# FlowEternal/multitask-hydranet

Hardware: AMD Instinct MI355X
Metric: images/sec (fwd+bwd) HydraNet @ default res, 1/2/4/8 MI355X; CPU-ref same run (higher is better)
Workload: dtype bf16; 1 GPU; full HydraNet (backbone + BiFPN + seg/det/lane heads + multitask loss), big cfg, fwd+loss+bwd; batch_per_gpu=16, global_batch=16, resolution=3x512x1024, parallelism=dp1, hipgraph=True

## Files before the change

### include/hydranet_hip.h

```cpp
#ifndef HYDRANET_HIP_H
#define HYDRANET_HIP_H

#ifdef __cplusplus
extern "C" {
#endif

typedef struct ihipStream_t* hipStream_t;


int hn_gconv_pack_diag(const float* w, void* wk, void* wd, int C, hipStream_t stream);
int hn_pack_weight(const float* w, void* wp, void* wt, int Cout, int Cin, int taps, hipStream_t stream);
int hn_pack_weight_ex(const float* w, void* wp, void* wt, int Cout, int Cin_total, int ci0, int Cin, int taps, int phase, const float* bias,
                      float* b_eff, hipStream_t stream);
int hn_phase_fold(const float* dw_eff, const float* dw1, const float* db_eff, float* dw, float* db, int K, int C0, int C1, hipStream_t stream);
int hn_pack_weights_batched(const long* jobs, int njobs, long total_blocks, const int* block_job, hipStream_t stream);
int hn_pack_small_batched(const long* jobs, const int* block_job, long total_blocks, hipStream_t stream);

int hn_conv_gemm_nt(const void* x0, const void* x1, int mode, int n_img, int H, int W, int C0, int C1, int ld0, int ld1, int up, long M,
                    const void* w, int Nout, int KP, int taps, const float* bias, int act, void* out, int out_f32, int ldc, long rpi,
                    long img_stride, float* psum, float* psq, hipStream_t stream);
int hn_nt_stat_rows(long M, int Nout);
int hn_nt_stat_tile(long M, int Nout);
int hn_conv_gemm_nt_stream(const void* x, int ld0, long M, int C0, const void* w, int Nout, int KP, const float* bias, int act, void* out,
                           int ldc, float* psum, float* psq, int wg_limit, hipStream_t stream);
int hn_nt_stream_ok(long M, int C0, int Nout, int KP);
int hn_direct_stat_rows(int n_img, int H, int W);
int hn_conv_gemm_nt_imgw(const void* x0, int ld0, long M, int C0, const void* w, long w_img_stride, long rows_per_image, int Nout, int KP,
                         const float* bias, int act, void* out, int ldc, const void* addend, int ld_add, hipStream_t stream);
int hn_scale_weight_gate(const void* wp, const float* gate, void* out, int N, int Cout, int C, int KP, hipStream_t stream);
int hn_conv_gemm_nt_lvl(const void* x0, int ld0, long M, int C0, const void* w, int Nout, int KP, const float* bias, int act, void* out,
                        int ldc, const float* coef, int nlev, const long* rows, hipStream_t stream);
int hn_conv_gemm_nt_lvlout(const void* x0, int ld0, long M, int C0, const void* w, int Nout, int KP, const float* bias, int act, float* out,
                           int ldc, long img_stride, int n_img, int nlev, const int* H, const int* W, int row_align, hipStream_t stream);

int hn_conv_gemm_nt_ex(const void* x0, const void* x1, int mode, int n_img, int H, int W, int C0, int C1, int ld0, int ld1, int up, long M,
                       const void* w, int Nout, int KP, int taps, const float* bias, int act, void* out, int out_f32, int ldc, long rpi,
                       long img_stride, float* psum, float* psq, const float* xscale, const float* xshift, const float* xgate, long xhw,
                       int xact, const void* addend, int ld_add, int add_mode, hipStream_t stream);
int hn_conv_gemm_nt_stat(const void* x0, const void* x1, int mode, int n_img, int H, int W, int C0, int C1, int ld0, int ld1, int up, long M,
                         const void* w, int Nout, int KP, int taps, const float* bias, int act, void* out, int out_f32, int ldc, long rpi,
                         long img_stride, float* psum, float* psq, const void* addend, int ld_add, int add_mode, int emode, const void* ez,
                         int ld_ez, const float* ecoef, hipStream_t stream);
int hn_conv_gemm_nt_stat3(const void* x0, int ld0, long M, int C0, const void* w, int Nout, int KP, void* out, int ldc, float* psum, float* psq,
                          const void* addend, int ld_add, const void* ez, int ld_ez, const void* ey, int ld_ey, const float* ecoef,
                          hipStream_t stream);
int hn_wgrad_plan(int mode, int n_img, int H, int W, long M, int Nout, int KP, int taps, int* splits, long* rows_per_split, long* ws_bytes);
int hn_conv_gemm_tn(const void* x0, const void* x1, int mode, int n_img, int H, int W, int C0, int C1, int ld0, int ld1, int up, long M,
                    const void* dz, int ldz, int Nout, int KP, int taps, float* workspace, float* dw, hipStream_t stream);


int hn_stem_fwd(const float* x, const float* w, void* z, void* patches, int N, int H, int W, hipStream_t stream);

int hn_gconv_pack(const float* w, void* wk, void* wd, int C, int flip, hipStream_t stream);
int hn_gconv_fwd(const void* in, int ldi, const void* wk, void* out, int ldo, int N, int Hi, int Wi, int C, int stride, hipStream_t stream);
int hn_gconv_dgrad_s2(const void* dz, int ldz, const void* wd, void* dx, int ldx, int N, int Hi, int Wi, int C, hipStream_t stream);
long hn_wgrad_chunks(long pixels, long items);
int hn_gconv_wgrad(const void* x, int ldx, const void* dz, int ldz, float* part, int N, int Hi, int Wi, int C, int stride,
                   hipStream_t stream);

int hn_dw_pack(const float* w, void* wk, void* wkf, int C, hipStream_t stream);
int hn_dwconv_fwd(const void* in, int ldi, const void* wk, void* out, int ldo, int N, int H, int W, int C, hipStream_t stream);
int hn_dwconv_fwd_levels(const void* in, int ldi, const void* wk, void* out, int ldo, int N, int C, int nlev, const int* H, const int* W,
                         int row_align, int accumulate, hipStream_t stream);
long hn_dwconv_wgrad_blocks(long strips, int C);
int hn_dwconv_wgrad(const void* x, int ldx, const void* dz, int ldz, float* part, int N, int H, int W, int C, hipStream_t stream);
int hn_dwconv_wgrad_levels(const void* x, int ldx, const void* dz, int ldz, float* part, int N, int C, int nlev, const int* H, const int* W,
                           int row_align, hipStream_t stream);
long hn_dwconv_bwd_blocks(long strips, int C);
long hn_dwconv_bwd_blocks_levels(int N, int C, int nlev, const int* H, const int* W);
int hn_dwconv_bwd_levels(const void* dz, int ldz, const void* x, int ldx, const void* wf, void* dx, int lddx, float* part, int N, int C,
                         int nlev, const int* H, const int* W, int row_align, int accumulate, hipStream_t stream);

int hn_maxpool_fwd(const void* in, int ldi, void* out, int ldo, int N, int H, int W, int C, int mode, hipStream_t stream);
int hn_maxpool_bwd(const void* in, int ldi, const void* dout, int ldd, void* dx, int ldx, const float* wscale, int N, int H, int W, int C,
                   int mode, hipStream_t stream);
int hn_maxpool_bwd2(const void* in, int ldi, const void* dout, int ldd, void* dx, int ldx, const float* wscale, void* arg_ws, int N, int H,
                    int W, int C, int mode, int accumulate, hipStream_t stream);

int hn_up2_fwd(const void* in, int ldi, void* out, int ldo, int N, int H, int W, int C, hipStream_t stream);
int hn_sum2x2(const void* g, int ldg, void* out, int ldo, const float* wscale, int N, int H, int W, int C, int accumulate, hipStream_t stream);

int hn_fuse_dweights(const float* pw, int blocks, const float* praw, int nw, float eps, float* dp, hipStream_t stream);
int hn_fuse_fwd(const void* const* in, const int* ld, const int* mode, const float* w, void* out, int ldo, int N, int H, int W, int C,
                hipStream_t stream);
int hn_fuse_fwd_raw(const void* const* in, const int* ld, const int* mode, const float* praw, int nw, float eps, float* wn, void* out, int ldo,
                    int N, int H, int W, int C, hipStream_t stream);
int hn_fuse_bwd_blocks(int N, int H, int W, int C);
int hn_fuse_bwd(const void* const* in, const int* ld, const int* mode, const float* w, const void* dout, int ldd, void* g, int ldg,
                void* const* din, const int* ldin, const int* acc, float* pw, int N, int H, int W, int C, hipStream_t stream);
int hn_fuse_bwd_arg(const void* const* in, const int* ld, const int* mode, const float* w, const void* dout, int ldd, void* g, int ldg,
                    void* const* din, const int* ldin, const int* acc, float* pw, void* const* arg_out, int N, int H, int W, int C,
                    hipStream_t stream);
int hn_maxpool_bwd_from_arg(const void* arg, const void* dout, int ldd, void* dx, int ldx, const float* wscale, int N, int H, int W, int C,
                            int mode, int accumulate, hipStream_t stream);

long hn_fold_ring_rows(int H, int W);
int hn_conv3x3_dgrad_fold(const void* dz, int ldz, int Cz, int n_img, int H, int W, const void* wt, int Nout, int KP, int phase_k, int clamp,
                          void* out, int ldo, const void* yprev, int ldy, void* ring, hipStream_t stream);
int hn_conv3x3_dgrad_fold_s2d(const void* dz, int ldz, int Cz, int n_img, int H, int W, const void* wt, int Nout, int KP, int phase_k, int clamp,
                              void* out, int ldo, void* out_s2d, int ld_s2d, const void* yprev, int ldy, void* ring, hipStream_t stream);
int hn_seg_fold(const void* dvp, int ldv, int c0, void* out, int ldo, const void* yprev, int ldy, int N, int H, int W, int C, int up,
                hipStream_t stream);

int hn_space_to_depth(const float* dy, void* out, int ldo, int N, int h, int w, int k, hipStream_t stream);

int hn_space_to_depth_blocks(int N, int h, int w, int k);
int hn_space_to_depth_bf16(const void* in, int ldi, void* out, int N, int h, int w, int k, float* psum, hipStream_t stream);

int hn_conv3x3_phase(const void* x0, int mode, int n_img, int H, int W, int C0, int ld0, const void* w, int Nout, int KP, const float* bias,
                     int act, void* out, int ldc, int k, const void* addend, int ld_add, hipStream_t stream);
int hn_conv3x3_out_argmax(const void* x0, int n_img, int H, int W, int C0, int ld0, const void* w, int k, int KP, const float* bias, long* mask,
                          hipStream_t stream);
int hn_wgrad_plan_phase(int n_img, int H, int W, int Nout, int KP, int phase_span, int* splits, long* rows_per_split, long* ws_bytes);
int hn_conv_gemm_tn_phase(const void* x0, int n_img, int H, int W, int C0, int ld0, const void* dz, int ldz, int Nout, int KP, int phase_span,
                          float* workspace, float* dw, float* dbias_eff, hipStream_t stream);
int hn_conv_gemm_tn_deferred(const void* x0, const void* x1, int mode, int n_img, int H, int W, int C0, int C1, int ld0, int ld1, int up, long M,
                             const void* dz, int ldz, int Nout, int KP, int taps, float* workspace, float* dw, long* job, hipStream_t stream);
int hn_wgrad_reduce_jobs(const long* jobs, int njobs, hipStream_t stream);
long hn_gconv_wgrad_group_ws_bytes(const long* jobs, int njobs);
int hn_gconv_wgrad_group(const long* jobs, int njobs, float* workspace, hipStream_t stream);

int hn_grad_tail(const long* jobs, int njobs, hipStream_t stream);

long hn_wgrad_group_ws_bytes(const long* jobs, int njobs);
int hn_wgrad_group(const long* jobs, int njobs, float* workspace, hipStream_t stream);

int hn_conv_gemm_tn_bias(const void* x0, const void* x1, int mode, int n_img, int H, int W, int C0, int C1, int ld0, int ld1, int up, long M,
                         const void* dz, int ldz, int Nout, int KP, int taps, float* workspace, float* dw, float* dbias, hipStream_t stream);

int hn_head_grad(const float* dy, const float* y, long rpi, long img_stride, int lds, int Nout, void* dz, int ldz, long M, int sigmoid,
                 hipStream_t stream);

int hn_pack_levels(const void* const* src, const int* ld, void* dst, int ldd, int N, int C, int nlev, const int* H, const int* W, int row_align,
                   hipStream_t stream);
int hn_head_grad_levels(const float* dy, const float* y, long img_stride, int lds, int Nout, void* dz, int ldz, int N, int nlev, const int* H,
                        const int* W, int row_align, int sigmoid, hipStream_t stream);


long hn_colred_rows(long M, long align);
int hn_col_stats(const void* x, int ldx, long M, int C, long R, float* psum, float* psq, hipStream_t stream);
int hn_col_dot(const void* a, int lda, const void* b, int ldb, long M, int C, long R, float* pdot, float* psum, hipStream_t stream);
int hn_rows_reduce(const float* in, float* out, int G, int S, int C, float alpha, hipStream_t stream);
int hn_rows_reduce2(const float* in1, const float* in2, float* out1, float* out2, int rows, int G, int C, hipStream_t stream);

int hn_bn_finalize(const float* psum, const float* psq, int prows, int C, long count, const float* gamma, const float* beta, float eps,
                   float momentum, float* running_mean, float* running_var, float* scale, float* shift, float* mean, float* rstd,
                   hipStream_t stream);
int hn_bn_eval_coeff(const float* gamma, const float* beta, const float* rm, const float* rv, float eps, int C, float* scale, float* shift,
                     hipStream_t stream);
int hn_bn_act(const void* z, int ldz, const float* scale, const float* shift, const void* res, int ldr, const float* rscale,
              const float* rshift, int act, void* out, int ldo, long M, int C, hipStream_t stream);
int hn_bn_bwd_reduce(const void* dout, int ldd, const void* z, int ldz, const void* y, int ldy, const float* scale, const float* shift,
                     const float* mean, const float* rstd, int act, long M, int C, long R, float* pg, float* pgx, hipStream_t stream);
int hn_bn_bwd_finalize(const float* pg, const float* pgx, int prows, int C, long count, float* dgamma, float* dbeta, float* mg, float* mgx,
// ... 301 lines not shown
```

### multitask_hydranet_amd/csrc/hn_stencil.hip

```cpp
#include "hn_common.h"

__global__ __launch_bounds__(256) void stem_fwd_kernel(const float* x, const float* w, bf16* z, bf16* patches, int N, int H, int W) {
    const int bidx = xcd_remap(blockIdx.x, gridDim.x);
    __shared__ float sw[27][32];
    for (int i = threadIdx.x; i < 27 * 32; i += 256) {
        const int co = i & 31, t = i >> 5;
        sw[t][co] = w[co * 27 + t];
    }
    __syncthreads();
    const int Ho = H >> 1, Wo = W >> 1, Wp = (Wo + 1) >> 1;
    const long total = (long)N * Ho * Wp;
    const long idx = (long)bidx * 256 + threadIdx.x;
    if (idx >= total) return;
    const int ox = (int)(idx % Wp) * 2;
    const long t1 = idx / Wp;
    const int oy = (int)(t1 % Ho);
    const long n = t1 / Ho;
    const bool two = ox + 1 < Wo;
    float acc[2][32];
#pragma unroll
    for (int c = 0; c < 32; ++c) { acc[0][c] = 0.f; acc[1][c] = 0.f; }
    __shared__ __attribute__((aligned(16))) bf16 sp[2][256][36];
    bf16* prow = patches ? sp[0][threadIdx.x] : nullptr;
    constexpr int PH = 256 * 36;
// ... 780 lines not shown
            const int px = (int)(((unsigned)e * magic) >> 16), pc = e - px * C8;
            const int py = px / 18, pxx = px - py * 18;
            const int iy = oy0 - 1 + py, ix = ox0 - 1 + pxx;
            const bf16* src = (px < ZPX && iy >= 0 && iy < H && ix >= 0 && ix < W) ? dz + (row0 + (long)iy * W + ix) * ldz + pc * 8 : st_zero_piece;
            st_glds16(src, sZ + ch * 1024);
        }
        for (int ch = wave; ch < XCH; ch += 4) {
            const int e = ch * 64 + lane;
            const int px = (int)(((unsigned)e * magic) >> 16), pc = e - px * C8;
            const int iy = oy0 + (px >> 4), ix = ox0 + (px & 15);
            const bf16* src = (px < XPX && iy < H && ix < W) ? x + (row0 + (long)iy * W + ix) * ldx + pc * 8 : st_zero_piece;
            st_glds16(src, sX + ch * 1024);
        }
        asm volatile("s_waitcnt vmcnt(0)" ::: "memory");
        __syncthreads();
        if (active)
#pragma unroll 1
        for (int col = colh; col < 16; col += 8) {
            bf16x4 win[3][3];
            auto load_row = [&](int py, bf16x4 (&w3)[3]) {
#pragma unroll
                for (int j = 0; j < 3; ++j) w3[j] = *reinterpret_cast<const bf16x4*>(sZ + ((py * 18 + col + j) * C4 + cq) * 8);
            };
            load_row(0, win[0]);
            load_row(1, win[1]);
#pragma unroll 1
            for (int r3 = 0; r3 < TH; r3 += 3)
#pragma unroll
            for (int rq = 0; rq < 3; ++rq) {
                const int r = r3 + rq;
                if (r >= TH) break;
                load_row(r + 2, win[(rq + 2) % 3]);
                const bf16x4 xb = *reinterpret_cast<const bf16x4*>(sX + ((r * 16 + col) * C4 + cq) * 8);
                float xv[4], da[4];
#pragma unroll
                for (int k = 0; k < 4; ++k) { xv[k] = bf2f(xb[k]); da[k] = 0.f; }
#pragma unroll
                for (int rr = 0; rr < 3; ++rr)
#pragma unroll
                    for (int j = 0; j < 3; ++j) {
                        const bf16x4 zq = win[(rq + rr) % 3][j];
#pragma unroll
                        for (int k = 0; k < 4; ++k) {
                            const float zf = bf2f(zq[k]);
                            if (HAS_DX) da[k] = fmaf(zf, wr[rr * 3 + j][k], da[k]);
                            acc[8 - (rr * 3 + j)][k] = fmaf(xv[k], zf, acc[8 - (rr * 3 + j)][k]);
                        }
                    }
                if (HAS_DX && oy0 + r < H && ox0 + col < W) {
                    bf16* dst = dx + (row0 + (long)(oy0 + r) * W + ox0 + col) * lddx + cq * 4;
                    bf16x4 v;
                    if (accumulate) {
                        const bf16x4 prev = ld4(dst);
#pragma unroll
                        for (int k = 0; k < 4; ++k) v[k] = f2bf(da[k] + bf2f(prev[k]));
                    } else {
#pragma unroll
                        for (int k = 0; k < 4; ++k) v[k] = f2bf(da[k]);
                    }
                    *reinterpret_cast<bf16x4*>(dst) = v;
                }
            }
        }
    }
    __syncthreads();
    float* red = reinterpret_cast<float*>(smem);
    if (active) {
#pragma unroll
        for (int tq = 0; tq < 9; ++tq)
#pragma unroll
            for (int k = 0; k < 4; ++k) red[(colh * C4 + cq) * 37 + tq * 4 + k] = acc[tq][k];
    }
    __syncthreads();
    float* dst = part + (long)bidx * C * 9;
    for (int o = tid; o < C4 * 36; o += 256) {
        const int g = o / 36, v = o - g * 36;
        float sum = 0.f;
#pragma unroll
        for (int c2 = 0; c2 < 8; ++c2) sum += red[(c2 * C4 + g) * 37 + v];
        dst[(long)(g * 4 + (v & 3)) * 9 + (v >> 2)] = sum;
    }
}

__global__ void dw_pack_kernel(const float* w, bf16* wk, bf16* wkf, int C) {
    const int idx = blockIdx.x * blockDim.x + threadIdx.x;
    if (idx >= 9 * C) return;
    const int c = idx % C, tap = idx / C;
    const bf16 v = f2bf(w[c * 9 + tap]);
    wk[idx] = v;
    if (wkf) wkf[(8 - tap) * C + c] = v;
}

__device__ __forceinline__ void pool_window(const bf16* in, int ldi, long n, int H, int W, int oy, int ox, int c, int mode, float* best,
                                            int* arg) {
#pragma unroll
    for (int k = 0; k < 8; ++k) { best[k] = -INFINITY; arg[k] = -1; }
    const int off = mode ? -1 : 0;
#pragma unroll
    for (int ky = 0; ky < 3; ++ky)
#pragma unroll
        for (int kx = 0; kx < 3; ++kx) {
            const int iy = 2 * oy + ky + off, ix = 2 * ox + kx + off;
            const bool inside = iy >= 0 && iy < H && ix >= 0 && ix < W;
            if (!inside && mode) continue;
            bf16x8 v = inside ? ld8(in + ((n * H + iy) * (long)W + ix) * ldi + c) : zero8();
#pragma unroll
            for (int k = 0; k < 8; ++k) {
                const float f = bf2f(v[k]);
                if (f > best[k]) { best[k] = f; arg[k] = inside ? ky * 3 + kx : 9; }
            }
        }
}

__global__ __launch_bounds__(256) void maxpool_fwd_kernel(const bf16* in, int ldi, bf16* out, int ldo, int N, int H, int W, int C,
                                                          int mode) {
    const int bidx = xcd_remap(blockIdx.x, gridDim.x);
    const int C8 = C >> 3, Ho = H >> 1, Wo = W >> 1;
    const long total = (long)N * Ho * Wo * C8;
    for (long idx = (long)bidx * 256 + threadIdx.x; idx < total; idx += (long)gridDim.x * 256) {
        const int cg = (int)(idx % C8);
        long t = idx / C8;
        const int ox = (int)(t % Wo);
        t /= Wo;
        const int oy = (int)(t % Ho);
        const long n = t / Ho;
        float best[8];
        int arg[8];
        pool_window(in, ldi, n, H, W, oy, ox, cg * 8, mode, best, arg);
        bf16x8 v;
#pragma unroll
        for (int k = 0; k < 8; ++k) v[k] = f2bf(best[k]);
        st8(out + ((n * Ho + oy) * (long)Wo + ox) * ldo + cg * 8, v);
    }
}

__global__ __launch_bounds__(256) void maxpool_bwd_kernel(const bf16* in, int ldi, const bf16* dout, int ldd, bf16* dx, int ldx,
                                                          const float* wscale, int N, int H, int W, int C, int mode) {
    const int bidx = xcd_remap(blockIdx.x, gridDim.x);
    const int C8 = C >> 3, Ho = H >> 1, Wo = W >> 1;
    const long total = (long)N * H * W * C8;
    const float ws = wscale ? *wscale : 1.0f;
    const int off = mode ? -1 : 0;
    for (long idx = (long)bidx * 256 + threadIdx.x; idx < total; idx += (long)gridDim.x * 256) {
        const int cg = (int)(idx % C8);
        long t = idx / C8;
        const int ix = (int)(t % W);
        t /= W;
        const int iy = (int)(t % H);
        const long n = t / H;
        float acc[8];
#pragma unroll
        for (int k = 0; k < 8; ++k) acc[k] = 0.f;
        for (int oy = (iy - off - 2 + 1) >> 1; 2 * oy + off <= iy; ++oy) {
            if (oy < 0 || oy >= Ho) continue;
            for (int ox = (ix - off - 2 + 1) >> 1; 2 * ox + off <= ix; ++ox) {
                if (ox < 0 || ox >= Wo) continue;
                float best[8];
                int arg[8];
                pool_window(in, ldi, n, H, W, oy, ox, cg * 8, mode, best, arg);
                const int mine = (iy - 2 * oy - off) * 3 + (ix - 2 * ox - off);
                const bf16x8 g = ld8(dout + ((n * Ho + oy) * (long)Wo + ox) * ldd + cg * 8);
#pragma unroll
                for (int k = 0; k < 8; ++k)
                    if (arg[k] == mine) acc[k] += bf2f(g[k]);
            }
        }
// ... 667 lines not shown
    const int lanes = 256 / (C >> 2);
    const long tb = g_hn_knob[7] > 0 ? g_hn_knob[7] : 768;
    long spl = (strips + (tb - 1) * lanes) / (tb * lanes);
    if (spl < 2) spl = 2;
    return (strips + spl * lanes - 1) / (spl * lanes);
}
extern "C" long hn_dwconv_bwd_blocks(long strips, int C) { return dwconv_bwd_strip_blocks(strips, C); }
static size_t dwconv_bwd_tiled_lds(int C8) {
    return (size_t)((((DWT_TH + 2) * 18 * C8 + 63) >> 6) + ((DWT_TH * 16 * C8 + 63) >> 6)) * 1024;
}
static bool dwconv_bwd_tiled_plan(int N, int C, const Levels& L, DwTiles& T, int& tpw, long& blocks) {
    T.tile_off[0] = 0;
    for (int l = 0; l < L.n; ++l) {
        T.ty[l] = (L.H[l] + DWT_TH - 1) / DWT_TH;
        T.tx[l] = (L.W[l] + 15) >> 4;
        T.tile_off[l + 1] = T.tile_off[l] + (long)N * T.ty[l] * T.tx[l];
    }
    const long total = T.tile_off[L.n];
    const int C8 = C >> 3;
    const size_t lds = dwconv_bwd_tiled_lds(C8);
#ifdef HN_NO_DW_TILED
    return false;
#endif
    if (g_hn_knob[7] < 0 || C8 > 16 || lds > 80 * 1024 || total < 512) return false;
    tpw = (int)((total + 511) / 512);
    blocks = (total + tpw - 1) / tpw;
    return true;
}
extern "C" long hn_dwconv_bwd_blocks_levels(int N, int C, int nlev, const int* H, const int* W) {
    Levels L;
    if (fill_levels(L, N, nlev, H, W) != HN_OK || (C & 7) || C < 8) return -1;
    DwTiles T;
    int tpw = 0;
    long blocks = 0;
    if (dwconv_bwd_tiled_plan(N, C, L, T, tpw, blocks)) return blocks;
    long strips = 0;
    for (int l = 0; l < nlev; ++l) strips += (long)N * H[l] * ((W[l] + 3) >> 2);
    return dwconv_bwd_strip_blocks(strips, C);
}
extern "C" int hn_dwconv_bwd_levels(const void* dz, int ldz, const void* x, int ldx, const void* wf, void* dx, int lddx, float* part, int N, int C,
                                    int nlev, const int* H, const int* W, int row_align, int accumulate, hipStream_t st) {
    Levels L;
    const int rc = fill_levels(L, N, nlev, H, W, row_align);
    if (rc != HN_OK) return rc;
    HN_CHECK_ARG(dz && x && part && (!dx || wf) && (C & 7) == 0 && C >= 8 && C <= 1024 && ((ldz | ldx) & 7) == 0 && (!dx || (lddx & 7) == 0));
    long pad_items = 0;
    if (dx && !accumulate)
        for (int l = 0; l < L.n; ++l) pad_items += (L.row_off[l + 1] - L.row_off[l] - (long)N * L.H[l] * L.W[l]) * (C >> 3);
    DwTiles T;
    int tpw = 0;
    long tblocks = 0;
    if (dwconv_bwd_tiled_plan(N, C, L, T, tpw, tblocks)) {
        const int C8 = C >> 3;
        const size_t lds = dwconv_bwd_tiled_lds(C8);
        if (lds > 64 * 1024) {
            static std::atomic<unsigned long long> optin_t{0};
            if (!lds_optin(optin_t, {(const void*)dwconv_bwd_tiled_kernel<true>, (const void*)dwconv_bwd_tiled_kernel<false>})) return HN_ERR_LAUNCH;
        }
        L.work_off[0] = 0;
        if (dx)
            hipLaunchKernelGGL(dwconv_bwd_tiled_kernel<true>, dim3((unsigned)(tblocks + cdiv(pad_items, 256))), dim3(256), lds, st, (const bf16*)dz,
                               ldz, (const bf16*)x, ldx, (const bf16*)wf, (bf16*)dx, lddx, part, N, C, tpw, (int)tblocks, L, T, accumulate);
        else
            hipLaunchKernelGGL(dwconv_bwd_tiled_kernel<false>, dim3((unsigned)tblocks), dim3(256), lds, st, (const bf16*)dz, ldz, (const bf16*)x, ldx,
                               (const bf16*)wf, (bf16*)dx, lddx, part, N, C, tpw, (int)tblocks, L, T, accumulate);
        HN_LAUNCH_CHECK();
    }
    L.work_off[0] = 0;
    for (int l = 0; l < L.n; ++l) L.work_off[l + 1] = L.work_off[l] + (long)N * L.H[l] * ((L.W[l] + 3) >> 2);
    const long strips = L.work_off[L.n];
    const int lanes = 256 / (C >> 2);
    const long blocks = dwconv_bwd_strip_blocks(strips, C);
    const int spl = (int)((strips + blocks * lanes - 1) / (blocks * lanes));
    const size_t lds = (256 * 37 + 9 * (size_t)C) * sizeof(float);
    if (lds > 64 * 1024) {
        static std::atomic<unsigned long long> optin{0};
        if (!lds_optin(optin, {(const void*)dwconv_bwd_kernel})) return HN_ERR_LAUNCH;
    }
    hipLaunchKernelGGL(dwconv_bwd_kernel, dim3((unsigned)(blocks + cdiv(pad_items, 256))), dim3(256), lds, st, (const bf16*)dz, ldz, (const bf16*)x,
                       ldx, (const bf16*)wf, (bf16*)dx, lddx, part, N, C, spl, blocks, L, accumulate);
    HN_LAUNCH_CHECK();
}

extern "C" int hn_maxpool_fwd(const void* in, int ldi, void* out, int ldo, int N, int H, int W, int C, int mode, hipStream_t st) {
    HN_CHECK_ARG(in && out && (C & 7) == 0 && ((ldi | ldo) & 7) == 0 && !(H & 1) && !(W & 1) && (mode == 0 || mode == 1));
    hipLaunchKernelGGL(maxpool_fwd_kernel, dim3(ew_grid((long)N * (H >> 1) * (W >> 1) * (C >> 3))), dim3(256), 0, st, (const bf16*)in, ldi,
                       (bf16*)out, ldo, N, H, W, C, mode);
    HN_LAUNCH_CHECK();
}
extern "C" int hn_maxpool_bwd(const void* in, int ldi, const void* dout, int ldd, void* dx, int ldx, const float* wscale, int N, int H,
                              int W, int C, int mode, hipStream_t st) {
    HN_CHECK_ARG(in && dout && dx && (C & 7) == 0 && ((ldi | ldd | ldx) & 7) == 0 && !(H & 1) && !(W & 1));
    hipLaunchKernelGGL(maxpool_bwd_kernel, dim3(ew_grid((long)N * H * W * (C >> 3))), dim3(256), 0, st, (const bf16*)in, ldi,
                       (const bf16*)dout, ldd, (bf16*)dx, ldx, wscale, N, H, W, C, mode);
    HN_LAUNCH_CHECK();
}
extern "C" int hn_maxpool_bwd2(const void* in, int ldi, const void* dout, int ldd, void* dx, int ldx, const float* wscale, void* arg_ws,
                               int N, int H, int W, int C, int mode, int accumulate, hipStream_t st) {
    HN_CHECK_ARG(in && dout && dx && arg_ws && (C & 7) == 0 && ((ldi | ldd | ldx) & 7) == 0 && !(H & 1) && !(W & 1));
    hipLaunchKernelGGL(maxpool_arg_kernel, dim3(ew_grid((long)N * (H >> 1) * (W >> 1) * (C >> 3))), dim3(256), 0, st, (const bf16*)in, ldi,
                       (unsigned char*)arg_ws, N, H, W, C, mode);
    hipLaunchKernelGGL(maxpool_bwd_arg_kernel, dim3(ew_grid((long)N * H * W * (C >> 3))), dim3(256), 0, st, (const unsigned char*)arg_ws,
                       (const bf16*)dout, ldd, (bf16*)dx, ldx, wscale, N, H, W, C, mode, accumulate);
    HN_LAUNCH_CHECK();
}
extern "C" int hn_maxpool_bwd_from_arg(const void* arg, const void* dout, int ldd, void* dx, int ldx, const float* wscale, int N, int H, int W,
                                       int C, int mode, int accumulate, hipStream_t st) {
    HN_CHECK_ARG(arg && dout && dx && (C & 7) == 0 && ((ldd | ldx) & 7) == 0 && !(H & 1) && !(W & 1));
    hipLaunchKernelGGL(maxpool_bwd_arg_kernel, dim3(ew_grid((long)N * H * W * (C >> 3))), dim3(256), 0, st, (const unsigned char*)arg,
                       (const bf16*)dout, ldd, (bf16*)dx, ldx, wscale, N, H, W, C, mode, accumulate);
    HN_LAUNCH_CHECK();
}
extern "C" int hn_up2_fwd(const void* in, int ldi, void* out, int ldo, int N, int H, int W, int C, hipStream_t st) {
    HN_CHECK_ARG(in && out && (C & 7) == 0 && ((ldi | ldo) & 7) == 0);
    hipLaunchKernelGGL(up2_fwd_kernel, dim3(ew_grid((long)N * 4 * H * W * (C >> 3))), dim3(256), 0, st, (const bf16*)in, ldi, (bf16*)out, ldo,
                       N, H, W, C);
    HN_LAUNCH_CHECK();
}
extern "C" int hn_sum2x2(const void* g, int ldg, void* out, int ldo, const float* wscale, int N, int H, int W, int C, int accumulate,
                         hipStream_t st) {
    HN_CHECK_ARG(g && out && (C & 7) == 0 && ((ldg | ldo) & 7) == 0);
    hipLaunchKernelGGL(sum2x2_kernel, dim3(ew_grid((long)N * H * W * (C >> 3))), dim3(256), 0, st, (const bf16*)g, ldg, (bf16*)out, ldo, wscale,
                       N, H, W, C, accumulate);
    HN_LAUNCH_CHECK();
}

static int fill_fuse(Fuse& f, const void* const* in, const int* ld, const int* mode, const float* w, void* out, int ldo, int N, int H,
                     int W, int C) {
    HN_CHECK_ARG(in && ld && mode && (C & 7) == 0 && (ldo & 7) == 0);
    for (int i = 0; i < 3; ++i) {
        f.in[i] = (const bf16*)in[i]; f.ld[i] = ld[i]; f.mode[i] = mode[i];
        HN_CHECK_ARG(mode[i] >= 0 && mode[i] <= 3 && (mode[i] == 0 || (in[i] && (ld[i] & 7) == 0)));
        HN_CHECK_ARG(mode[i] != 2 || (!(H & 1) && !(W & 1)));
    }
    f.w = w; f.out = (bf16*)out; f.ldo = ldo; f.N = N; f.H = H; f.W = W; f.C = C;
    f.praw = nullptr; f.nw = 0; f.eps = 0.f; f.wn = nullptr;
    return HN_OK;
}
extern "C" int hn_fuse_fwd(const void* const* in, const int* ld, const int* mode, const float* w, void* out, int ldo, int N, int H, int W,
                           int C, hipStream_t st) {
    Fuse f;
    HN_CHECK_ARG(out);
    const int rc = fill_fuse(f, in, ld, mode, w, out, ldo, N, H, W, C);
    if (rc) return rc;
    hipLaunchKernelGGL(fuse_fwd_kernel, dim3(ew_grid((long)N * H * W * (C >> 3))), dim3(256), 0, st, f);
    HN_LAUNCH_CHECK();
}
extern "C" int hn_fuse_fwd_raw(const void* const* in, const int* ld, const int* mode, const float* praw, int nw, float eps, float* wn,
                               void* out, int ldo, int N, int H, int W, int C, hipStream_t st) {
    Fuse f;
    HN_CHECK_ARG(out && praw && wn && nw >= 1 && nw <= 3);
    const int rc = fill_fuse(f, in, ld, mode, nullptr, out, ldo, N, H, W, C);
    if (rc) return rc;
    f.praw = praw; f.nw = nw; f.eps = eps; f.wn = wn;
    hipLaunchKernelGGL(fuse_fwd_kernel, dim3(ew_grid((long)N * H * W * (C >> 3))), dim3(256), 0, st, f);
    HN_LAUNCH_CHECK();
}
extern "C" int hn_fuse_bwd_blocks(int N, int H, int W, int C) {
    long b = ((long)N * H * W * (C >> 3) + 255) / 256;
    if (b > 1024) b = 1024;
    return (int)(b < 1 ? 1 : b);
}
extern "C" int hn_fuse_bwd(const void* const* in, const int* ld, const int* mode, const float* w, const void* dout, int ldd, void* g,
                           int ldg, void* const* din, const int* ldin, const int* acc, float* pw, int N, int H, int W, int C,
                           hipStream_t st) {
    FuseBwd q;
// ... 146 lines not shown
```

### multitask_hydranet_amd/ops/neck.py

```python
from __future__ import annotations

import ctypes
import os
from typing import Optional, Sequence, Tuple

import torch

from .._lib import lib, policy
from .core import *
from .backbone import *


def k_dwconv(x, wk, out=None):
    n, h, w, c = x.shape
    if out is None:
        out = new_act(n, h, w, c, x.device)
    lib().call("hn_dwconv_fwd", ptr(x), ld(x), ptr(wk), ptr(out), ld(out), n, h, w, c)
    return out


def k_dwconv_wgrad(x, dz):
    n, h, w, c = x.shape
    chunks = lib().query("hn_dwconv_wgrad_blocks", n * h * ((w + 3) // 4), c)
    part = torch.empty((chunks, c * 9), device=x.device, dtype=F32)
    lib().call("hn_dwconv_wgrad", ptr(x), ld(x), ptr(dz), ld(dz), ptr(part), n, h, w, c)
    return k_rows_reduce(part, 1, chunks, c * 9).view(c, 1, 3, 3)


def k_dwconv_bwd(dz, x, wf, geom=None, want_dx=True, into=None, queue=None, weight=None):
    c = x.shape[3]
    if geom is None:
        n, h, w, _ = x.shape
        H, W, nl, align = (ctypes.c_int * 1)(h), (ctypes.c_int * 1)(w), 1, 1
    else:
        nl, H, W, _, _ = _geom_arrays(geom)
        n, align = geom[0], LEVEL_ALIGN
    blocks = lib().query("hn_dwconv_bwd_blocks_levels", n, c, nl, ctypes.addressof(H), ctypes.addressof(W))
    part = torch.empty((blocks, c * 9), device=x.device, dtype=F32)
    dx = None
    if want_dx:
        dx = torch.empty_like(dz) if into is None else into
    lib().call("hn_dwconv_bwd_levels", ptr(dz), ld(dz), ptr(x), ld(x), ptr(wf), ptr(dx), ld(dx) if dx is not None else 0, ptr(part), n, c, nl,
               ctypes.addressof(H), ctypes.addressof(W), align, 0 if into is None else 1)
    if queue is not None:
        queue.add_rows(weight, part, blocks, c * 9, (c, 1, 3, 3))
        return dx, None
    return dx, k_rows_reduce(part, 1, blocks, c * 9).view(c, 1, 3, 3)


class DwConv(torch.autograd.Function):
    @staticmethod
    def forward(ctx, x, weight):
        wk, wf = pack_dw_weight(weight)
        ctx.queue, ctx.wref = (cur_queue() if weight.requires_grad else None), weight
        ctx.save_for_backward(x, wf)
        return k_dwconv(x, wk)

    @staticmethod
    def backward(ctx, dout):
        x, wf = ctx.saved_tensors
        dout = dense(dout)
        return k_dwconv_bwd(dout, x, wf, want_dx=ctx.needs_input_grad[0], queue=ctx.queue, weight=ctx.wref)


def k_maxpool(x, mode, out=None):
    n, h, w, c = x.shape
    if out is None:
        out = new_act(n, h // 2, w // 2, c, x.device)
    lib().call("hn_maxpool_fwd", ptr(x), ld(x), ptr(out), ld(out), n, h, w, c, mode)
    return out


def k_maxpool_bwd(x, dout, mode, wscale=None, into=None, accumulate=False):
    n, h, w, c = x.shape
    dx = new_act(n, h, w, c, x.device) if into is None else into
    arg = torch.empty((n * (h // 2) * (w // 2) * c,), device=x.device, dtype=torch.uint8)
    lib().call("hn_maxpool_bwd2", ptr(x), ld(x), ptr(dout), ld(dout), ptr(dx), ld(dx), ptr(wscale), ptr(arg), n, h, w, c, mode,
               1 if accumulate else 0)
    return dx


class MaxPool(torch.autograd.Function):
    @staticmethod
    def forward(ctx, x, mode):
        ctx.mode = mode
        ctx.save_for_backward(x)
        return k_maxpool(x, mode)

    @staticmethod
    def backward(ctx, dout):
        (x,) = ctx.saved_tensors
        return k_maxpool_bwd(x, dense(dout), ctx.mode), None


def _fuse_args(ins, modes):
    arr_p = (ctypes.c_void_p * 3)(*[ptr(t) if t is not None else None for t in ins])
    arr_l = (ctypes.c_int * 3)(*[ld(t) if t is not None else 0 for t in ins])
    arr_m = (ctypes.c_int * 3)(*modes)
    return arr_p, arr_l, arr_m


class GradSlot:
    __slots__ = ("buf",)

    def __init__(self):
        self.buf = None


class Share(torch.autograd.Function):

    @staticmethod
    def forward(ctx, x, slot, n):
        ctx.slot = slot
        ctx.set_materialize_grads(False)
        return tuple(x.view_as(x) for _ in range(n))

    @staticmethod
    def backward(ctx, *grads):
        buf, ctx.slot.buf = ctx.slot.buf, None
        gs = [dense(g) for g in grads if g is not None]
        if buf is None and gs:
            buf = gs.pop(0)
            if gs and buf.data_ptr() in [g.data_ptr() for g in gs]:
                buf = buf.clone()
        while gs:
            part, gs = gs[:3], gs[3:]
# ... 90 lines not shown
```

Before: 995.2 images/sec.

## Add channel-split tiled depthwise conv backward kernel for small-tile levels

Adds a depthwise-conv backward kernel that splits channels into chunks across blocks and tiles spatially with halo-staged LDS. It is used when the total tile count is small (256 or fewer), so that small BiFPN levels expose more parallelism. The per-tile weight-grad partials are written as rows, so the reduction row count changes. The cost is extra halo reloads per chunk and an extra code path.

```diff
diff --git a/include/hydranet_hip.h b/include/hydranet_hip.h
--- a/include/hydranet_hip.h
+++ b/include/hydranet_hip.h
@@ -70,6 +70,10 @@
 long hn_dwconv_bwd_blocks_levels(int N, int C, int nlev, const int* H, const int* W);
 int hn_dwconv_bwd_levels(const void* dz, int ldz, const void* x, int ldx, const void* wf, void* dx, int lddx, float* part, int N, int C,
                          int nlev, const int* H, const int* W, int row_align, int accumulate, hipStream_t stream);
+long hn_dwconv_bwd_split_rows(int N, int C, int nlev, const int* H, const int* W);
+int hn_dwconv_bwd_split_chunk(int N, int C, int nlev, const int* H, const int* W);
+int hn_dwconv_bwd_split_levels(const void* dz, int ldz, const void* x, int ldx, const void* wf, void* dx, int lddx, float* part, int N, int C,
+                               int nlev, const int* H, const int* W, int row_align, int accumulate, int chunk, hipStream_t stream);
 
 int hn_maxpool_fwd(const void* in, int ldi, void* out, int ldo, int N, int H, int W, int C, int mode, hipStream_t stream);
 int hn_maxpool_bwd(const void* in, int ldi, const void* dout, int ldd, void* dx, int ldx, const float* wscale, int N, int H, int W, int C,
diff --git a/multitask_hydranet_amd/csrc/hn_stencil.hip b/multitask_hydranet_amd/csrc/hn_stencil.hip
--- a/multitask_hydranet_amd/csrc/hn_stencil.hip
+++ b/multitask_hydranet_amd/csrc/hn_stencil.hip
@@ -886,6 +886,148 @@
     }
 }
 
+template <bool HAS_DX>
+__global__ __launch_bounds__(256, 2) void dwconv_bwd_split_kernel(const bf16* dz, int ldz, const bf16* x, int ldx, const bf16* wf, bf16* dx, int lddx,
+                                                                  float* part, int N, int C, int CC, int blocks, const Levels L, const DwTiles T,
+                                                                  int accumulate) {
+    extern __shared__ __attribute__((aligned(16))) char smem[];
+    constexpr int TH = DWT_TH;
+    const int C8 = C >> 3, C4c = CC >> 2;
+    const int tid = threadIdx.x, lane = tid & 63, wave = __builtin_amdgcn_readfirstlane(tid >> 6);
+    if ((int)blockIdx.x >= blocks) {
+        long idx = ((long)blockIdx.x - blocks) * 256 + tid;
+        for (int l = 0; l < L.n; ++l) {
+            const long real = (long)N * L.H[l] * L.W[l];
+            const long pad = L.row_off[l + 1] - L.row_off[l] - real;
+            if (idx < pad * C8) {
+                st8(dx + (L.row_off[l] + real + idx / C8) * lddx + (idx % C8) * 8, zero8());
+                return;
+            }
+            idx -= pad * C8;
+        }
+        return;
+    }
+    const int chunks = C / CC;
+    const int bidx = xcd_remap(blockIdx.x, blocks);
+    const long t = bidx / chunks;
+    const int c0 = (bidx - (int)t * chunks) * CC;
+    const int a0 = c0 & ~7, P = ((c0 + CC + 7) >> 3) - (a0 >> 3);
+    const int coff = (c0 - a0) >> 2;
+    int lv = 0;
+    while (lv + 1 < L.n && t >= T.tile_off[lv + 1]) ++lv;
+    const int H = L.H[lv], W = L.W[lv];
+    long lt = t - T.tile_off[lv];
+    const int tx = (int)(lt % T.tx[lv]);
+    lt /= T.tx[lv];
+    const int ty = (int)(lt % T.ty[lv]);
+    const long n = lt / T.ty[lv];
+    const int oy0 = ty * TH, ox0 = tx * 16;
+    const int th = H - oy0 < TH ? H - oy0 : TH, tw = W - ox0 < 16 ? W - ox0 : 16;
+    const long row0 = L.row_off[lv] + n * H * (long)W;
+    const int ZPX = (th + 2) * 18, XPX = th * 16;
+    const int ZCH = (ZPX * P + 63) >> 6, XCH = (XPX * P + 63) >> 6;
+    char* sZ = smem;
+    char* sX = smem + ZCH * 1024;
+    const int lanes = 256 / C4c;
+    const int CL = lanes >= 16 ? 16 : 8;
+    int RS = 1;
+    while (RS < TH && CL * RS * 2 <= lanes) RS *= 2;
+    const int NL = CL * RS, RPS = TH / RS;
+    const int cq = tid % C4c, ln = tid / C4c;
+    const bool active = ln < NL;
+    const int colh = ln % CL, rbase = (ln / CL) * RPS;
+    const int rend = rbase + RPS < th ? rbase + RPS : th;
+    float wr[9][4], acc[9][4];
+#pragma unroll
+    for (int tq = 0; tq < 9; ++tq) {
+        const bf16x4 wv = (HAS_DX && active) ? ld4(wf + tq * C + c0 + cq * 4) : zero4();
+#pragma unroll
+        for (int k = 0; k < 4; ++k) { wr[tq][k] = bf2f(wv[k]); acc[tq][k] = 0.f; }
+    }
+    const unsigned magic = (65536u + P - 1) / P;
+    for (int ch = wave; ch < ZCH; ch += 4) {
+        const int e = ch * 64 + lane;
+        const int px = (int)(((unsigned)e * magic) >> 16), pc = e - px * P;
+        const int py = px / 18, pxx = px - py * 18;
+        const int iy = oy0 - 1 + py, ix = ox0 - 1 + pxx;
+        const bf16* src = (px < ZPX && iy >= 0 && iy < H && ix >= 0 && ix < W) ? dz + (row0 + (long)iy * W + ix) * ldz + a0 + pc * 8 : st_zero_piece;
+        st_glds16(src, sZ + ch * 1024);
+    }
+    for (int ch = wave; ch < XCH; ch += 4) {
+        const int e = ch * 64 + lane;
+        const int px = (int)(((unsigned)e * magic) >> 16), pc = e - px * P;
+        const int iy = oy0 + (px >> 4), ix = ox0 + (px & 15);
+        const bf16* src = (px < XPX && iy < H && ix < W) ? x + (row0 + (long)iy * W + ix) * ldx + a0 + pc * 8 : st_zero_piece;
+        st_glds16(src, sX + ch * 1024);
+    }
+    asm volatile("s_waitcnt vmcnt(0)" ::: "memory");
+    __syncthreads();
+    if (active && rbase < rend)
+#pragma unroll 1
+    for (int col = colh; col < tw; col += CL) {
+        bf16x4 win[3][3];
+        auto load_row = [&](int py, bf16x4 (&w3)[3]) {
+#pragma unroll
+            for (int j = 0; j < 3; ++j) w3[j] = *reinterpret_cast<const bf16x4*>(sZ + (((py * 18 + col + j) * P * 2) + coff + cq) * 8);
+        };
+        load_row(rbase, win[0]);
+        load_row(rbase + 1, win[1]);
+#pragma unroll 1
+        for (int r3 = rbase; r3 < rend; r3 += 3)
+#pragma unroll
+        for (int rq = 0; rq < 3; ++rq) {
+            const int r = r3 + rq;
+            if (r >= rend) break;
+            load_row(r + 2, win[(rq + 2) % 3]);
+            const bf16x4 xb = *reinterpret_cast<const bf16x4*>(sX + (((r * 16 + col) * P * 2) + coff + cq) * 8);
+            float xv[4], da[4];
+#pragma unroll
+            for (int k = 0; k < 4; ++k) { xv[k] = bf2f(xb[k]); da[k] = 0.f; }
+#pragma unroll
+            for (int rr = 0; rr < 3; ++rr)
+#pragma unroll
+                for (int j = 0; j < 3; ++j) {
+                    const bf16x4 zq = win[(rq + rr) % 3][j];
+#pragma unroll
+                    for (int k = 0; k < 4; ++k) {
+                        const float zf = bf2f(zq[k]);
+                        if (HAS_DX) da[k] = fmaf(zf, wr[rr * 3 + j][k], da[k]);
+                        acc[8 - (rr * 3 + j)][k] = fmaf(xv[k], zf, acc[8 - (rr * 3 + j)][k]);
+                    }
+                }
+            if (HAS_DX) {
+                bf16* dst = dx + (row0 + (long)(oy0 + r) * W + ox0 + col) * lddx + c0 + cq * 4;
+                bf16x4 v;
+                if (accumulate) {
+                    const bf16x4 prev = ld4(dst);
+#pragma unroll
+                    for (int k = 0; k < 4; ++k) v[k] = f2bf(da[k] + bf2f(prev[k]));
+                } else {
+#pragma unroll
+                    for (int k = 0; k < 4; ++k) v[k] = f2bf(da[k]);
+                }
+                *reinterpret_cast<bf16x4*>(dst) = v;
+            }
+        }
+    }
+    __syncthreads();
+    float* red = reinterpret_cast<float*>(smem);
+    if (active) {
+#pragma unroll
+        for (int tq = 0; tq < 9; ++tq)
+#pragma unroll
+            for (int k = 0; k < 4; ++k) red[(ln * C4c + cq) * 37 + tq * 4 + k] = acc[tq][k];
+    }
+    __syncthreads();
+    float* dst = part + t * C * 9 + (long)c0 * 9;
+    for (int o = tid; o < C4c * 36; o += 256) {
+        const int g = o / 36, v = o - g * 36;
+        float sum = 0.f;
+        for (int l = 0; l < NL; ++l) sum += red[(l * C4c + g) * 37 + v];
+        dst[(long)(g * 4 + (v & 3)) * 9 + (v >> 2)] = sum;
+    }
+}
+
 __global__ void dw_pack_kernel(const float* w, bf16* wk, bf16* wkf, int C) {
     const int idx = blockIdx.x * blockDim.x + threadIdx.x;
     if (idx >= 9 * C) return;
@@ -1719,6 +1861,75 @@
     HN_LAUNCH_CHECK();
 }
 
+static bool dwconv_bwd_split_chunk_ok(int C, int CC) { return CC >= 4 && (CC & 3) == 0 && C % CC == 0 && C / CC <= 4 && C / CC != 3; }
+static long dwconv_bwd_split_tiles(int N, const Levels& L, DwTiles& T) {
+    T.tile_off[0] = 0;
+    for (int l = 0; l < L.n; ++l) {
+        T.ty[l] = (L.H[l] + DWT_TH - 1) / DWT_TH;
+        T.tx[l] = (L.W[l] + 15) >> 4;
+        T.tile_off[l + 1] = T.tile_off[l] + (long)N * T.ty[l] * T.tx[l];
+    }
+    return T.tile_off[L.n];
+}
+extern "C" long hn_dwconv_bwd_split_rows(int N, int C, int nlev, const int* H, const int* W) {
+    Levels L;
+    DwTiles T;
+    if (fill_levels(L, N, nlev, H, W) != HN_OK || (C & 7) || C < 8 || C > 128) return -1;
+    const long tiles = dwconv_bwd_split_tiles(N, L, T);
+    return tiles <= (1L << 20) ? tiles : -1;
+}
+extern "C" int hn_dwconv_bwd_split_chunk(int N, int C, int nlev, const int* H, const int* W) {
+    const long tiles = hn_dwconv_bwd_split_rows(N, C, nlev, H, W);
+    if (tiles < 0) return -1;
+    int best = C;
+    for (int k = 2; k <= 4; k <<= 1) {
+        if (!dwconv_bwd_split_chunk_ok(C, C / k) || C % k) break;
+        if (tiles * (C / best) >= 512) break;
+        best = C / k;
+    }
+    return best;
+}
+extern "C" int hn_dwconv_bwd_split_levels(const void* dz, int ldz, const void* x, int ldx, const void* wf, void* dx, int lddx, float* part, int N,
+                                          int C, int nlev, const int* H, const int* W, int row_align, int accumulate, int chunk, hipStream_t st) {
+    Levels L;
+    const int rc = fill_levels(L, N, nlev, H, W, row_align);
+    if (rc != HN_OK) return rc;
+    HN_CHECK_ARG(dz && x && part && (!dx || wf) && (C & 7) == 0 && C >= 8 && C <= 128 && ((ldz | ldx) & 7) == 0 && (!dx || (lddx & 7) == 0));
+    const int CC = chunk ? chunk : hn_dwconv_bwd_split_chunk(N, C, nlev, H, W);
+    HN_CHECK_ARG(dwconv_bwd_split_chunk_ok(C, CC));
+    DwTiles T;
+    const long tiles = dwconv_bwd_split_tiles(N, L, T);
+    HN_CHECK_ARG(tiles <= (1L << 20));
+    const int chunks = C / CC;
+    long pad_items = 0;
+    if (dx && !accumulate)
+        for (int l = 0; l < L.n; ++l) pad_items += (L.row_off[l + 1] - L.row_off[l] - (long)N * L.H[l] * L.W[l]) * (C >> 3);
+    int P = 0;
+    for (int k = 0; k < chunks; ++k) {
+        const int c0 = k * CC, p = ((c0 + CC + 7) >> 3) - (c0 >> 3);
+        if (p > P) P = p;
+    }
+    const int C4c = CC >> 2, lanes = 256 / C4c, CL = lanes >= 16 ? 16 : 8;
+    int RS = 1;
+    while (RS < DWT_TH && CL * RS * 2 <= lanes) RS *= 2;
+    const size_t tile = (size_t)((((DWT_TH + 2) * 18 * P + 63) >> 6) + ((DWT_TH * 16 * P + 63) >> 6)) * 1024;
+    const size_t fold = (size_t)CL * RS * C4c * 37 * sizeof(float);
+    const size_t lds = tile > fold ? tile : fold;
+    if (lds > 64 * 1024) {
+        static std::atomic<unsigned long long> optin_s{0};
+        if (!lds_optin(optin_s, {(const void*)dwconv_bwd_split_kernel<true>, (const void*)dwconv_bwd_split_kernel<false>})) return HN_ERR_LAUNCH;
+    }
+    L.work_off[0] = 0;
+    const long blocks = tiles * chunks;
+    if (dx)
+        hipLaunchKernelGGL(dwconv_bwd_split_kernel<true>, dim3((unsigned)(blocks + cdiv(pad_items, 256))), dim3(256), lds, st, (const bf16*)dz, ldz,
+                           (const bf16*)x, ldx, (const bf16*)wf, (bf16*)dx, lddx, part, N, C, CC, (int)blocks, L, T, accumulate);
+    else
+        hipLaunchKernelGGL(dwconv_bwd_split_kernel<false>, dim3((unsigned)blocks), dim3(256), lds, st, (const bf16*)dz, ldz, (const bf16*)x, ldx,
+                           (const bf16*)wf, (bf16*)dx, lddx, part, N, C, CC, (int)blocks, L, T, accumulate);
+    HN_LAUNCH_CHECK();
+}
+
 extern "C" int hn_maxpool_fwd(const void* in, int ldi, void* out, int ldo, int N, int H, int W, int C, int mode, hipStream_t st) {
     HN_CHECK_ARG(in && out && (C & 7) == 0 && ((ldi | ldo) & 7) == 0 && !(H & 1) && !(W & 1) && (mode == 0 || mode == 1));
     hipLaunchKernelGGL(maxpool_fwd_kernel, dim3(ew_grid((long)N * (H >> 1) * (W >> 1) * (C >> 3))), dim3(256), 0, st, (const bf16*)in, ldi,
diff --git a/multitask_hydranet_amd/ops/neck.py b/multitask_hydranet_amd/ops/neck.py
--- a/multitask_hydranet_amd/ops/neck.py
+++ b/multitask_hydranet_amd/ops/neck.py
@@ -27,7 +27,20 @@
     return k_rows_reduce(part, 1, chunks, c * 9).view(c, 1, 3, 3)
 
 
-def k_dwconv_bwd(dz, x, wf, geom=None, want_dx=True, into=None, queue=None, weight=None):
+DW_SPLIT = policy("HN_DW_SPLIT", "1") != "0"
+DW_SPLIT_MAX_TILES = 256
+
+
+def dw_split_rows(n, c, nl, H, W, split=None):
+    if not (DW_SPLIT if split is None else split):
+        return 0
+    rows = lib().query("hn_dwconv_bwd_split_rows", n, c, nl, ctypes.addressof(H), ctypes.addressof(W))
+    if rows <= 0:
+        return 0
+    return rows if split or rows <= DW_SPLIT_MAX_TILES else 0
+
+
+def k_dwconv_bwd(dz, x, wf, geom=None, want_dx=True, into=None, queue=None, weight=None, split=None, chunk=0):
     c = x.shape[3]
     if geom is None:
         n, h, w, _ = x.shape
@@ -35,13 +48,16 @@
     else:
         nl, H, W, _, _ = _geom_arrays(geom)
         n, align = geom[0], LEVEL_ALIGN
-    blocks = lib().query("hn_dwconv_bwd_blocks_levels", n, c, nl, ctypes.addressof(H), ctypes.addressof(W))
+    blocks = dw_split_rows(n, c, nl, H, W, split)
+    entry, tail = ("hn_dwconv_bwd_split_levels", (chunk,)) if blocks else ("hn_dwconv_bwd_levels", ())
+    if not blocks:
+        blocks = lib().query("hn_dwconv_bwd_blocks_levels", n, c, nl, ctypes.addressof(H), ctypes.addressof(W))
     part = torch.empty((blocks, c * 9), device=x.device, dtype=F32)
     dx = None
     if want_dx:
         dx = torch.empty_like(dz) if into is None else into
-    lib().call("hn_dwconv_bwd_levels", ptr(dz), ld(dz), ptr(x), ld(x), ptr(wf), ptr(dx), ld(dx) if dx is not None else 0, ptr(part), n, c, nl,
-               ctypes.addressof(H), ctypes.addressof(W), align, 0 if into is None else 1)
+    lib().call(entry, ptr(dz), ld(dz), ptr(x), ld(x), ptr(wf), ptr(dx), ld(dx) if dx is not None else 0, ptr(part), n, c, nl,
+               ctypes.addressof(H), ctypes.addressof(W), align, 0 if into is None else 1, *tail)
     if queue is not None:
         queue.add_rows(weight, part, blocks, c * 9, (c, 1, 3, 3))
         return dx, None
```

Result: no change. 1000.0 images/sec, median of 6 (+0.5%).
